# gt1/daccord

Measured on AMD Instinct MI355X. Metric: corrected Mbase/s (whole node), synthetic 20x PacBio piles, higher is better.
Workload: dtype u64+f64; 1 GPU; BASELINE.json configs[1] (10k A-reads x 10 kb x 20x, k=14, one MI355X): synthetic 10000 A-reads x 10000 b x 20x, 15% error (ins 80/del 13.3/sub 6.7), k=14, w=40, a=10, tspace=100; piles_total=10000, piles_rank0=10000, overlaps_rank0=319252, windows_rank0=9969965, trace_blocks_rank0=17906701, corrected_bases_total=90715992

## Files before the change

daccord_amd/csrc/capi.hip:

```cpp
#include <hip/hip_runtime.h>
#include <vector>
#include <string>
#include <cstring>
#include <cstdio>
#include <cstdlib>
#include <new>
#include "../../include/daccord_hip.h"
#include "batch_plan.hpp"
#include "host_tables.hpp"
#include "window_kernels.hpp"
#include "trace_kernel.hpp"
#include "vote_kernel.hpp"
#include "emit_record.hpp"

using namespace dacc;


struct PrepBatch
{
	DevOvl const * ovl; uint64_t novl; uint8_t const * trace; uint32_t trace_bytes;
	uint32_t * blk_ovl; uint32_t * blk_b0;
};

__global__ void k_prep(PrepBatch B)
// ... 323 lines not shown
	std::vector<uint32_t> h_rlen;
	BatchPlan BP;
	DevBuf<DevPile> d_piles; DevBuf<DevOvl> d_ovl; DevBuf<uint32_t> d_ovl_pile; DevBuf<uint8_t> d_trace;
	DevBuf<uint32_t> d_blk_ovl, d_blk_b0, d_wt_b, d_wt_e;
	DevBuf<uint8_t> d_wrec; DevBuf<WindowOut> d_wout; DevBuf<uint8_t> d_arena;
	DevBuf<uint8_t> d_has, d_oc, d_outsym, d_pilebad; DevBuf<uint16_t> d_ld0; DevBuf<uint32_t> d_ocs, d_nfrag, d_err;
	DevBuf<VoteFragment> d_frags; DevBuf<uint64_t> d_fragbase; DevBuf<uint64_t> d_prof;
	DevBuf<uint64_t> d_vst; DevBuf<uint32_t> d_tab32; DevBuf<uint8_t> d_gslab, d_longslab ; DevBuf<uint32_t> d_longhand[2];  DevBuf<uint32_t> d_retry[TIER_NSLOTS], d_work, d_gearly, d_pregen, d_pregen2, d_pregenlist; DevBuf<uint8_t> d_arena2; DevBuf<uint64_t> d_trslab; DevBuf<uint32_t> d_small; DevBuf<uint64_t> d_hand; DevBuf<uint32_t> d_handctr; uint32_t handcap; uint64_t handwant, nruns; bool nohand, oom; bool tier7_adapt_off; int env_t7adapt; int env_trdyn;
	TierSwitches sw; TierPipeline TP;
	struct Stage { bool ran; uint32_t grid; DevBuf<uint32_t> handon; DevBuf<uint8_t> slab; hipEvent_t done; uint32_t const * in;  } st[TIER_NSTAGES];
	uint32_t nlong[2];
	bool longran[2]; hipEvent_t evLong[4];
	uint32_t retry_grid, early_grid; int sched;
	uint32_t tr_grid, tr_lds, tr_words, tr_lanes, trace_bytes, win_grid;
	int env_sched, env_dbgretry;
	std::vector<uint32_t> retry_flags;
	std::vector<dacc_fragment> frags; std::string bases;
	std::vector<int32_t> pile_status; std::vector<std::string> pile_errors; std::string pile_errors_joined;
	std::vector<uint32_t> h_nfrag; std::vector<VoteFragment> h_frags; HostBuf<uint8_t> h_outsym;
	dacc_timing timing;
};

#define HIPCHK(call) do { hipError_t const e_ = (call); if ( e_ != hipSuccess ) { c->err = std::string(#call) + ": " + hipGetErrorString(e_); if ( e_ == hipErrorOutOfMemory ) c->oom = true; return DACC_EHIP; } } while (0)

template<typename T>
static int upload(dacc_ctx * c, DevBuf<T> & b, T const * src, size_t n)
{
	HIPCHK(b.ensure(n ? n : 1));
	if ( n ) HIPCHK(hipMemcpyAsync(b.p,src,n*sizeof(T),hipMemcpyHostToDevice,c->stream));
	return DACC_OK;
// ... 28 lines not shown
	if ( hipGetDeviceCount(&ndev) != hipSuccess || ndev <= 0 || p->device < 0 || p->device >= ndev )
		return DACC_ENODEV;
	if ( hipSetDevice(p->device) != hipSuccess ) return DACC_ENODEV;
	dacc_ctx * c = new (std::nothrow) dacc_ctx;
	if ( !c ) return DACC_ENOMEM;
	c->par = *p; c->device = p->device; c->haveprofile = c->havedb = c->havebatch = false; c->est_cor = 0; c->nlong[0] = c->nlong[1] = 0; c->longran[0] = c->longran[1] = false; c->handcap = 0; c->handwant = 0; c->nruns = 0; c->nohand = false; c->oom = false;
	std::memset(&c->timing,0,sizeof(c->timing));
	c->retry_grid = c->early_grid = c->win_grid = 0; c->tier7_adapt_off = false; c->sched = 0;
	c->tr_grid = c->tr_lds = c->tr_words = c->tr_lanes = c->trace_bytes = 0;
	{
		c->sw = readTierSwitches();
		char const * sc = getenv("DACC_SCHED"); c->env_sched = sc ? atoi(sc) : 1;
		{ char const * td = getenv("DACC_TRACE_DYN"); c->env_trdyn = !(td && td[0] == '0'); }
		char const * ta = getenv("DACC_T7_ADAPT"); c->env_t7adapt = !(ta && ta[0] == '0');
		char const * dr = getenv("DACC_DEBUG_RETRY"); c->env_dbgretry = (dr && dr[0] == '1');
	}
	if ( hipStreamCreate(&c->stream) != hipSuccess ) { delete c; return DACC_EHIP; }
	{ int lo = 0, hi = 0; hipDeviceGetStreamPriorityRange(&lo,&hi); if ( hipStreamCreateWithPriority(&c->stream2,hipStreamNonBlocking,hi) != hipSuccess ) { delete c; return DACC_EHIP; } }
	hipEventCreateWithFlags(&c->evFirstTier,hipEventDisableTiming); hipEventCreateWithFlags(&c->evEarlyGeneric,hipEventDisableTiming); hipEventCreateWithFlags(&c->evPrescan,hipEventDisableTiming);
	for ( int i = 0; i < 6; ++i ) hipEventCreate(&c->ev[i]);
	for ( int i = 0; i < 2; ++i ) hipEventCreate(&c->evEmit[i]);
	for ( int i = 0; i < 4; ++i ) hipEventCreate(&c->evLong[i]);
	for ( int i = 0; i < TIER_NSLOTS; ++i ) hipEventCreate(&c->evslot[i]);
	for ( int i = 0; i < TIER_NSTAGES; ++i ) { hipEventCreate(&c->st[i].done); c->st[i].ran = false; c->st[i].grid = 0; c->st[i].in = 0; }
	*out = c;
	return DACC_OK;
}

void dacc_destroy(dacc_ctx * c)
{
// ... 127 lines not shown
		WB.pregen = 0;
		for ( uint32_t i = 0; i < TIER_NSTAGES; ++i ) c->st[i].ran = false;
		if ( TP.usefast && TP.anytier() )
		{
			HIPCHK(hipMemsetAsync(c->d_pregen.p,0,((BP.nwindows+31)/32+1)*sizeof(uint32_t),s));
			HIPCHK(hipMemsetAsync(c->d_pregen2.p,0,((BP.nwindows+31)/32+1)*sizeof(uint32_t),s));
			HIPCHK(hipMemsetAsync(c->d_pregenlist.p,0,sizeof(uint32_t),s));
			for ( int i = 0; i < TIER_NSLOTS; ++i ) HIPCHK(hipMemsetAsync(c->d_retry[i].p,0,sizeof(uint32_t),s));
			if ( BP.ovl.size() )
			{
				hipLaunchKernelGGL(k_prescan,dim3((BP.ovl.size()+3)/4),dim3(256),0,s,c->d_ovl.p,static_cast<uint64_t>(BP.ovl.size()),c->d_ovl_pile.p,c->d_piles.p,c->d_wt_b.p,c->d_wt_e.p,c->d_pregen.p,c->d_pregen2.p,TP.widetier ? 128u : 64u);
				hipLaunchKernelGGL(k_prescan_lists,dim3(((BP.nwindows+31)/32+255)/256),dim3(256),0,s,c->d_pregen.p,c->d_pregen2.p,static_cast<uint64_t>(BP.nwindows),c->d_pregenlist.p,
					TP.slot1_long ? c->d_retry[0].p : static_cast<uint32_t *>(0),c->d_wout.p);
			}
			HIPCHK(hipEventRecord(c->evPrescan,s));
			FastBatch FL; FL.W = WB; FL.W.arena = c->d_arena2.p; FL.W.prof = 0; FL.W.pregen = 0; FL.F = BP.stageCaps(ID_LONG); FL.dpsq_vst = c->d_vst.p; FL.retry = 0; FL.gearly = 0; FL.gslab = 0; FL.gstride = 0; FL.tab32 = c->d_tab32.p; FL.hand = 0; FL.handctr = 0; FL.handcap = 0; FL.handwords = 0;
#if defined(DACC_LEDGER)
			FL.ledger = 0;
#endif
			bool const long5 = TP.ok[ID_LONG] && TP.tier[ID_LONG] == 5;
			if ( TP.tier[ID_LONG] != 5 ) FL.F = tierCaps(5,c->H.nrows,c->H.nsup);
			if ( !long5 ) FL.F.ldsbytes = 0;
			auto const launchLong = [&](uint32_t const * const lst, uint32_t & nlist, hipEvent_t const filled, uint32_t const which) -> int
			{
				nlist = 0;
				HIPCHK(hipStreamWaitEvent(c->stream2,filled,0));
				HIPCHK(hipMemcpyAsync(&nlist,lst,sizeof(uint32_t),hipMemcpyDeviceToHost,c->stream2));
				HIPCHK(hipStreamSynchronize(c->stream2));
				if ( !nlist ) return DACC_OK;
				uint32_t const * glist = lst;
				if ( TP.ok[ID_LONG] && TP.tier[ID_LONG] != 5 )
// ... 32 lines not shown
			HIPCHK(hipMemsetAsync(c->d_gearly.p,0,sizeof(uint32_t),s));
			HIPCHK(hipMemsetAsync(c->d_handctr.p,0,sizeof(uint32_t),s));
			bool early = false;
			HIPCHK(hipMemsetAsync(c->d_work.p,0,WORK_LONGSTR*sizeof(uint32_t),s));
			auto const work = [&](uint32_t const off) { return (c->sched&1) ? c->d_work.p+off : static_cast<uint32_t *>(0); };
			uint32_t const * list = 0; int lastslot = -1;
			FastBatch FZ;
			for ( uint32_t slot = 0; slot < TIER_NSLOTS; ++slot )
			{
				if ( TP.slotok(slot) )
				{
					int const m = TIER_MAIN[slot];
					FastBatch FB; FB.W = WB; FB.F = BP.stageCaps(m); FB.dpsq_vst = c->d_vst.p; FB.retry = c->d_retry[slot].p;
					if ( (slot > 0 && TP.late_long) || TP.widetier ) FB.W.pregen = c->d_pregen2.p;
					FB.gslab = c->d_gslab.p; FB.gstride = FB.F.gbytes; FB.tab32 = c->d_tab32.p;
					FB.hand = c->handcap ? c->d_hand.p : static_cast<uint64_t *>(0); FB.handctr = c->d_handctr.p; FB.handcap = c->handcap; FB.handwords = TP.handwords;
#if defined(DACC_LEDGER)
					{ char const * lm = getenv("DACC_LEDGER_MASK"); FB.ledger = lm ? static_cast<uint32_t>(strtoul(lm,0,0)) : 0u; }
#endif
					FB.gearly = early ? static_cast<uint32_t *>(0) : c->d_gearly.p;
					int fr[TIER_NSTAGES]; uint32_t nfr = 0;
					for ( int i = 0; i < m; ++i ) if ( TIER_CHAIN[i].slot == slot && TP.ok[i] && !((TIER_CHAIN[i].flags & STAGE_ADAPTIVE) && c->tier7_adapt_off) ) fr[nfr++] = i;
					bool const classed = nfr && (TIER_CHAIN[fr[0]].flags & STAGE_PREPASS);
					if ( classed ) HIPCHK(hipMemsetAsync(c->d_small.p,0,sizeof(uint32_t),s));
					for ( uint32_t k = 0; k < nfr; ++k ) HIPCHK(hipMemsetAsync(c->st[fr[k]].handon.p,0,sizeof(uint32_t),s));
					uint32_t const * in = list;
					if ( classed )
					{
						uint32_t * const mid = c->st[fr[0]].handon.p, * const big = c->st[fr[nfr-1]].handon.p;
						hipLaunchKernelGGL(k_classify,dim3((BP.nwindows+255)/256),dim3(256),0,s,WB,c->d_small.p,mid,big,c->sw.t0inst,nfr > 1 ? c->sw.t7inst : 0u);
						if ( nfr > 1 ) { HIPCHK(hipMemcpyAsync(c->d_work.p+WORK_PRE_MID,mid,sizeof(uint32_t),hipMemcpyDeviceToDevice,s)); HIPCHK(hipMemcpyAsync(c->d_work.p+WORK_PRE_BIG,big,sizeof(uint32_t),hipMemcpyDeviceToDevice,s)); }
// ... 501 lines not shown
```

daccord_amd/csrc/fast_window.hpp:

```cpp
#ifndef DACC_FAST_WINDOW_HPP
#define DACC_FAST_WINDOW_HPP
#include "wave.hpp"
#include "dev_types.hpp"
#include "arena.hpp"
#include "window_main.hpp"
#include "tier_pipeline.hpp"
#include "emit_record.hpp"

namespace dacc {

enum { WS_RETRY = 4 };
enum { FNOPAR = 0xFF };
enum { FSEQCAP = 48 };

struct FSI { uint64_t w; uint16_t left, right, current, path; };
struct FCC { uint64_t w; uint32_t o, l; };

template<int TIER> struct FastTier;
#if !defined(DACC_RCH01)
#define DACC_RCH01 2
#endif
template<> struct FastTier<1> { typedef uint8_t id_t; typedef uint8_t sid_t; enum : uint32_t { smax = 250, gw = 1, wcapg = 1024, rch = DACC_RCH01, fch = 4, fnw = 2, fnc = 40, idmax = 250, rpstcap = 256, lstr = 64, maxs = 32, precap = 1024, ncap = 776, scap = 112, lcap = 960, wcap = 1024, rccap = 144, fcap = 192, siqcap = 56, blcap = 96, seqcap = 32, psiq = 8, consrow = 64, lscrids = 2048, wide = 0, mins = 0, gmem = 0 }; };
template<> struct FastTier<0> { typedef uint8_t id_t; typedef uint8_t sid_t; enum : uint32_t { smax = 250, gw = 1, wcapg = 768, rch = DACC_RCH01, fch = 4, fnw = 2, fnc = 32, idmax = 250, rpstcap = 256, lstr = 64, maxs = 28, precap = 576, ncap = 524, scap = 88, lcap = 640, wcap = 768, rccap = 96, fcap = 128, siqcap = 56, blcap = 96, seqcap = 32, psiq = 8, consrow = 64, lscrids = 2048, wide = 0, mins = 0, gmem = 0 }; };
template<> struct FastTier<7> { typedef uint8_t id_t; typedef uint8_t sid_t; enum : uint32_t { smax = 250, gw = 1, wcapg = 896, rch = DACC_RCH01, fch = 4, fnw = 2, fnc = 32, idmax = 250, rpstcap = 256, lstr = 64, maxs = 28, precap = 704, ncap = 640, scap = 104, lcap = 800, wcap = 896, rccap = 112, fcap = 148, siqcap = 56, blcap = 96, seqcap = 32, psiq = 8, consrow = 64, lscrids = 2048, wide = 0, mins = 0, gmem = 0 }; };
// ... 401 lines not shown
	static_assert(CT::gmem == 0 || CT::gw != 0,"a layout in device memory is the gw layout");
	return C;
}

struct FastBatch
{
	WindowBatch W;
	FastCaps F;
	uint64_t const * dpsq_vst;
	uint32_t * retry;
	uint32_t * gearly;
	uint8_t * gslab;
	uint64_t gstride;
	uint32_t const * tab32;
	uint64_t * hand; uint32_t * handctr; uint32_t handcap, handwords;
#if defined(DACC_LEDGER)
	uint32_t ledger;
#endif
};

template<typename CT>
DEV void fast_load_tables(FastLds<CT> const & L, uint32_t const nrows, uint32_t const nsup, DevTables const & T, uint64_t const * vst)
{
	int const lane = wv_lane();
	for ( uint32_t i = lane; i < nsup; i += WSZ ) { L.suplo8()[i] = T.suplo[i]; L.suphi8()[i] = T.suphi[i]; }
	wv_sync();
}

#if defined(DACC_LEDGER)
#define LEDGER_REP(bit) for ( uint32_t lrep_ = 0, lrn_ = 1u + ((ledger >> (bit)) & 1u); lrep_ < lrn_; ++lrep_ )
// ... 32 lines not shown
	for ( size_t i = 0; i < it.size(); ++i ) tot += it[i];
	for ( size_t i = 0; i < it.size(); i += 64 ) { uint32_t m = 0; for ( size_t q = i; q < it.size() && q < i+64; ++q ) m = std::max(m,it[q]); lock += m; }
	std::vector< std::pair<uint32_t,uint32_t> > P; for ( size_t i = 0; i < it.size(); ++i ) P.push_back(std::make_pair(ln[i],it[i]));
	std::stable_sort(P.begin(),P.end(),[](std::pair<uint32_t,uint32_t> const & a, std::pair<uint32_t,uint32_t> const & b){ return a.first > b.first; });
	for ( size_t i = 0; i < P.size(); i += 64 ) { uint32_t m = 0; for ( size_t q = i; q < P.size() && q < i+64; ++q ) m = std::max(m,P[q].second); locksorted += m; }
	uint64_t lockcls = 0;
	{
		std::vector< std::pair<uint32_t,uint32_t> > Q; for ( size_t i = 0; i < it.size(); ++i ) { uint32_t c = 0; while ( (2u<<c) <= ln[i] ) ++c; Q.push_back(std::make_pair(c,it[i])); }
		std::stable_sort(Q.begin(),Q.end(),[](std::pair<uint32_t,uint32_t> const & a, std::pair<uint32_t,uint32_t> const & b){ return a.first > b.first; });
		for ( size_t i = 0; i < Q.size(); i += 64 ) { uint32_t m = 0; for ( size_t q = i; q < Q.size() && q < i+64; ++q ) m = std::max(m,Q[q].second); lockcls += m; }
	}
	fprintf(f,"%zu %llu %llu %llu %llu\n",it.size(),(unsigned long long)tot,(unsigned long long)lock,(unsigned long long)locksorted,(unsigned long long)lockcls);
	g_feasit.clear();
}
static inline bool feasit_on() { static int on = -1; if ( on < 0 ) on = getenv("DACC_EMUL_FEAS") ? 1 : 0; return on == 1; }
#define FEAS_ITERS(t,len,n) { if ( feasit_on() ) { g_feasit.it.push_back(n); g_feasit.ln.push_back(len); } }
#define FEAS_DUMP() { if ( feasit_on() ) feasit_dump(); }
struct FeasCases
{
	enum { NU = 0, NCU, NTASK, EMPTY_FIRST, EMPTY_MID, EMPTY_LAST, START_AT_ROUND, START_AT_ROUND_END, SPANS_ROUNDS, ROUNDS, LENMASK, MAXLEN, AT_CLAMP, PAST_CLAMP, MULTI, FAIL0, FAIL1, FAILLAST, NODES, N };
	uint64_t v[N];
	void clear() { for ( int i = 0; i < N; ++i ) v[i] = 0; }
	template<typename PT> void units(PT W, uint32_t const nu)
	{
		clear();
		v[NU] = nu;
		uint32_t first = nu, last = 0;
		for ( uint32_t q = 0; q < nu; ++q ) if ( W[q] ) { if ( first == nu ) first = q; last = q; }
		uint64_t t = 0;
		for ( uint32_t q = 0; q < nu; ++q )
		{
			uint32_t const w = W[q];
// ... 12 lines not shown
		if ( j == 0 ) { v[LENMASK] |= 1ull << (len < 63 ? len : 63); if ( len > v[MAXLEN] ) v[MAXLEN] = len; }
		if ( pp+1 == nrows ) ++v[AT_CLAMP];
		if ( pp >= nrows ) ++v[PAST_CLAMP];
		if ( f > 1 ) ++v[MULTI];
	}
	void fail(uint32_t const j, uint32_t const len) { if ( j == 0 ) ++v[FAIL0]; if ( j == 1 ) ++v[FAIL1]; if ( j+1 == len && len > 2 ) ++v[FAILLAST]; }
	void dump(int const tier, uint32_t const nwF, uint32_t const nwR)
	{
		static FILE * f = 0; static bool tried = false;
		if ( !tried ) { tried = true; char const * fn = getenv("DACC_EMUL_FEASCASES"); if ( fn ) f = fopen(fn,"w"); }
		if ( !f ) return;
		fprintf(f,"%d",tier); for ( int i = 0; i < N; ++i ) fprintf(f," %llu",(unsigned long long)v[i]); fprintf(f," %u %u\n",nwF,nwR); fflush(f);
	}
};
static FeasCases g_feascases;
#define FEAS_UNITS(W,nu) { if ( lane == 0 ) g_feascases.units(W,nu); }
#define FEAS_NODE(j,len,pp,nrows,f) g_feascases.node(j,len,pp,nrows,f);
#define FEAS_FAIL(j,len) g_feascases.fail(j,len);
#define FEAS_CASES_DUMP() { if ( lane == 0 ) g_feascases.dump(int(CT::maxs),nwF,nwR); }
#else
#define FEAS_ITERS(t,len,n)
#define FEAS_DUMP()
#define FEAS_UNITS(W,nu)
#define FEAS_NODE(j,len,pp,nrows,f)
#define FEAS_FAIL(j,len)
#define FEAS_CASES_DUMP()
#define FSTAT_MX(i,x)
#define FSTAT_ADD(i,x)
#endif

template<typename CT>
struct FastEngine
{
	typedef typename CT::id_t id_t;
	typedef typename CT::sid_t sid_t;
	enum : uint32_t { SB = 8u*sizeof(sid_t), SMASK = (1u<<SB)-1u, SNONE = SMASK, SMAX = CT::smax };
	FastLds<CT> L; DevTables T; DevParams P;
	uint32_t nrows, nsup;
	uint64_t const * vst;
	enum : bool { GW = (CT::gw != 0) };
	uint8_t * gslab;
	uint32_t const * gtab;
	struct G4 { uint32_t x, y, z, w; };
	int lane; uint32_t flags;
#if defined(DACC_LEDGER)
	uint32_t ledger;
#endif
	uint64_t * prof;
	uint32_t mao, k; uint64_t kmask;
	uint32_t npre, nlast, nn, nmfirst, nmlast;
	uint32_t n0, npool, nlinks, nwF, nwR;
	uint32_t nF, nL;

#if defined(DACC_EMUL)
	DEV void over_(uint32_t b, int line) { flags |= b; static char const * ov = getenv("DACC_EMUL_OVER"); if ( ov ) fprintf(stderr,"[over] tier maxs=%d line %d bits 0x%x nn=%u n0=%u npool=%u nF=%u nL=%u nwF=%u nwR=%u rstop=%u\n",int(CT::maxs)*10000+int(CT::ncap),line,b,nn,n0,npool,nF,nL,nwF,nwR,rstop); }
	#define over(b) over_(b,__LINE__)
#else
	DEV void over(uint32_t b) { flags |= b; }
#endif
#if defined(DACC_PROFILE) && !defined(DACC_EMUL)
	DEV void pcount(int id, uint64_t v) { if ( prof ) atomicAdd(reinterpret_cast<unsigned long long *>(prof+id),static_cast<unsigned long long>(v)); }
	DEV uint64_t pclock() { return clock64(); }
#else
	DEV void pcount(int, uint64_t) {}
	DEV uint64_t pclock() { return 0; }
#endif

#if defined(DACC_PROFILE) && !defined(DACC_EMUL)
// ... 785 lines not shown
			uint32_t const z = L.lnode()[c], par = L.parL()[c];
			if ( z == 0xFFFF ) continue;
			if ( par == SNONE ) ok |= reachN[z];
			else
			{
				ok |= vis[par];
				uint32_t const pl = L.posL()[c];
				for ( uint32_t f = 0; f < nF; ++f ) if ( L.parF()[f] == par && L.posF()[f] < pl ) ok = 1;
			}
		}
		bool const res = wv_any(ok) != 0;
		wv_sync();
		return res;
	}

	DEV void loadTab()
	{
		if constexpr ( GW ) return;
		else {
		uint32_t const stride = nrows+1;
		uint32_t pos = static_cast<uint32_t>(lane) / stride, row = static_cast<uint32_t>(lane) - pos*stride;
		uint32_t const dpos = WSZ / stride, drow = WSZ - dpos*stride;
		for ( uint32_t i = lane; i < stride*(nsup+1); i += WSZ )
		{
			L.tab()[i] = (row < nrows && pos < nsup) ? static_cast<uint32_t>(vst[pos*nrows+row]) : 0u;
			pos += dpos; row += drow; if ( row >= stride ) { row -= stride; ++pos; }
		}
		wv_sync();
		}
	}
	DEV uint32_t tabR(uint32_t const idx) const
	{
		if constexpr ( GW ) return gtab[idx];
		else return L.tab()[idx];
	}
	DEV auto unitRecords() const
	{
		if constexpr ( GW ) return L.urec();
		else { static_assert(2*CT::scap < 512,"unit ids are packed into 9 bits of a 16 bit record"); return reinterpret_cast<LDSQ uint16_t *>(L.ulo()); }
	}
	DEV void computeStretchFeasLanes(uint32_t const sfrom, uint32_t const sto)
	{
		PROFX_T0
		uint32_t const ns = sto-sfrom, nu = 2*ns;
		uint32_t const stride = nrows+1;
		enum { NCHU = (2*CT::scap + WSZ - 1)/WSZ, NCLS = 12 };
		typedef typename FastLds<CT>::toff_t toff_t;
		enum : uint32_t { TOFFMAX = sizeof(toff_t) == 2 ? 0xFFFFu : 0xFFFFFFu };
		static_assert(sizeof(toff_t) == 2 || 2ull*CT::scap*128ull <= TOFFMAX,"task offsets: every (stretch, direction, position) triple can be named");
		auto const urec = unitRecords();
		uint32_t ulo_r[NCHU], uw_r[NCHU], ucls_r[NCHU], upos_r[NCHU];
		#pragma unroll
		for ( uint32_t cc = 0; cc < NCHU; ++cc )
		{
			uint32_t const u = cc*WSZ + lane;
			uint32_t w = 0, lo_ = 0, cls = NCLS;
			if ( u < nu )
			{
				bool const rev = u >= ns; uint32_t const s = sfrom + (rev ? u-ns : u);
				uint32_t const len = L.sslen()[s]; LDSQ uint16_t const * Lk = L.links() + L.slink()[s];
				int32_t lo = 0, hi = static_cast<int32_t>(nrows);
				uint32_t const sh = rev ? 16 : 0;
				for ( uint32_t j = 0; j < len; ++j )
				{
					uint32_t const g = L.nrange()[Lk[rev ? (len-1-j) : j]] >> sh;
					int32_t const jj = static_cast<int32_t>(j);
					int32_t const a = static_cast<int32_t>(g&0xFF)-jj, b = static_cast<int32_t>((g>>8)&0xFF)-jj;
					lo = a > lo ? a : lo; hi = b < hi ? b : hi;
				}
				if ( hi < lo ) hi = lo;
				w = static_cast<uint32_t>(hi-lo); lo_ = static_cast<uint32_t>(lo);
				cls = len >= 49 ? 0u : len >= 33 ? 1u : len >= 25 ? 2u : len >= 17 ? 3u : len >= 13 ? 4u : len >= 9 ? 5u : len >= 7 ? 6u : len >= 5 ? 7u : len == 4 ? 8u : len == 3 ? 9u : len == 2 ? 10u : 11u;
				if ( rev ) { L.maskR()[s] = 0; L.woffR()[s] = 0; } else { L.maskF()[s] = 0; L.woffF()[s] = 0; }
				if constexpr ( CT::wide != 0 ) { if ( rev ) L.maskRh()[s] = 0; else L.maskFh()[s] = 0; }
			}
			ulo_r[cc] = lo_; uw_r[cc] = w; ucls_r[cc] = cls; upos_r[cc] = 0;
		}
		{
			uint32_t run = 0;
			for ( uint32_t k = 0; k < NCLS; ++k )
			{
				#pragma unroll
				for ( uint32_t cc = 0; cc < NCHU; ++cc )
				{
					if ( cc*WSZ >= nu ) break;
					bool const mine = ucls_r[cc] == k;
					uint32_t tot; uint32_t const pre = wv_scan_flag(mine,tot);
					if ( mine ) upos_r[cc] = run + pre;
					run += tot;
				}
			}
		}
		#pragma unroll
		for ( uint32_t cc = 0; cc < NCHU; ++cc )
		{
			uint32_t const u = cc*WSZ + lane;
			if ( u < nu ) { urec[upos_r[cc]] = ulo_r[cc] | (u << 7); L.toff()[upos_r[cc]] = static_cast<toff_t>(uw_r[cc]); }
		}
		wv_sync();
		FEAS_UNITS(L.toff(),nu)
		uint32_t tbase = 0;
		uint32_t ncu = 0;
		for ( uint32_t c = 0; c < nu; c += WSZ )
		{
			uint32_t const q = c + lane;
			uint32_t const w = q < nu ? L.toff()[q] : 0u;
			uint32_t const r = q < nu ? urec[q] : 0u;
			uint32_t tot; uint32_t const pre = wv_scan_excl(w,tot);
			uint32_t ntot; uint32_t const npre = wv_scan_flag(w != 0,ntot);
			if ( w != 0 ) { urec[ncu+npre] = r; L.toff()[ncu+npre] = static_cast<toff_t>(tbase + pre); }
			tbase += tot; ncu += ntot;
		}
		PROFX(18)
		if ( tbase > TOFFMAX ) { over(128); return; }
		if ( lane == 0 ) L.toff()[ncu] = static_cast<toff_t>(tbase);
		wv_sync();
		uint32_t const ntask = tbase;
		uint64_t const ltmask = wv_lanemask_lt();
		uint32_t ubase = 0;
		for ( uint32_t c = 0; c < ntask; c += WSZ )
		{
			uint32_t const t = c + lane;
			bool const act = t < ntask;
			uint32_t u = 0;
			{
				uint32_t const qi = ubase + 1u + static_cast<uint32_t>(lane);
				uint32_t const d = static_cast<uint32_t>(L.toff()[qi < ncu ? qi : ncu]) - c - 1u;
				uint64_t const starts = wv_or64(d < static_cast<uint32_t>(WSZ) ? (1ull << d) : 0ull);
				u = ubase + dacc_popc64(starts & ltmask);
// ... 38 lines not shown
					}
					FEAS_NODE(j,len,pp,nrows,f_a)
					if ( U < FW_THRES_FEAS ) { ok = false; FEAS_ITERS(t,len,j+1) FEAS_FAIL(j,len) break; }
					sum += U;
					if ( j == 0 ) f1 = U;
					fl = U;
					i0_a = i0_b; f_a = f_b; U_a = U_b; i0_b = i0_c; f_b = f_c; ip_b = ip_c; i0_c = i0_d; f_c = f_d; z_d = z_e;
				}
				if ( ok ) { FEAS_ITERS(t,len,len) }
				#undef DACC_LKN
			}
			uint64_t const okb = wv_ballot(ok);
			uint64_t const revb = wv_ballot(act && rev);
			uint64_t const mydir = rev ? revb : ~revb;
			uint32_t const base = rev ? nwR : nwF;
			if ( ok )
			{
				uint32_t const o = base + dacc_popc64(okb & mydir & ltmask);
				if ( o < CT::wcap )
				{
					if ( rev ) putR(o,sum,f1); else putF(o,sum,f1,fl);
				}
			}
			if ( act )
			{
				uint32_t const firstlane = (t0 > c) ? (t0-c) : 0u;
				if ( static_cast<uint32_t>(lane) == firstlane )
				{
					uint32_t const tend = L.toff()[u+1];
					uint32_t const lastlane = (tend-c < WSZ) ? (tend-c) : static_cast<uint32_t>(WSZ);
					uint64_t const span = (lastlane-firstlane >= 64) ? ~0ull : ((1ull << (lastlane-firstlane))-1ull);
					if constexpr ( CT::wide != 0 )
					{
						uint64_t const seg = (okb >> firstlane) & span;
						uint64_t const blo = P < 64u ? (seg << P) : 0ull, bhi = P < 64u ? (P ? (seg >> (64u-P)) : 0ull) : (seg << (P-64u));
						if ( rev ) { L.maskR()[s] |= blo; L.maskRh()[s] |= bhi; } else { L.maskF()[s] |= blo; L.maskFh()[s] |= bhi; }
					}
					else
					{
					uint64_t const bits = ((okb >> firstlane) & span) << P;
					if ( rev ) L.maskR()[s] |= bits; else L.maskF()[s] |= bits;
					}
					if ( t == t0 ) { uint32_t const wo = base + dacc_popc64(okb & mydir & ltmask); if ( rev ) L.woffR()[s] = wo; else L.woffF()[s] = wo; }
				}
			}
			nwF += dacc_popc64(okb & ~revb); nwR += dacc_popc64(okb & revb);
			if ( nwF > CT::wcap || nwR > CT::wcap ) { over(128); FEAS_DUMP() return; }
		}
		FEAS_DUMP()
		wv_sync();
		FEAS_CASES_DUMP()
	}
	enum : uint32_t { FQMAX = FastLds<CT>::fqmax, NWHB = FQMAX <= 255u ? 8u : (FQMAX <= 1023u ? 10u : 12u), NWHMASK = (1u << NWHB) - 1u,
		SWHB = FQMAX <= 1023u ? 16u : 18u, SWHMASK = (1u << SWHB) - 1u };
	static_assert((static_cast<uint64_t>(FQMAX)*0xFFFFFFFFull) >> (32u+NWHB) == 0,"high part of a node weight: fqmax table words");
	static_assert((64ull*static_cast<uint64_t>(FQMAX)*0xFFFFFFFFull) >> (32u+SWHB) == 0,"high part of a stretch weight: 64 nodes");
	static_assert(SWHB + NWHB <= 32u,"reverse record: both high parts in its third word");
	static_assert(SWHB == 16u || FastLds<CT>::wides,"a stretch weight of more than 48 bits needs the 32 byte forward record");
	static_assert(CT::maxs <= 1024 || (FastLds<CT>::fqmax == 4095u && FastLds<CT>::icap == 8u*CT::precap && FastLds<CT>::xwides),"more than 1024 strings: the widths of FastLds<CT>::xwides");
	static_assert(FastLds<CT>::wides || 16u + 2u*NWHB <= 32u,"forward record: three high parts in its fourth word, or the 32 byte record");
	struct G8 { G4 a, b; };
	struct WF { uint64_t w, w1, wl; };
	struct WR { uint64_t w, w1; };
	DEV WF recF(uint32_t const i) const
	{
		WF r;
// ... 71 lines not shown
	{
		if ( p >= nrows ) return 0;
		uint32_t const i0 = L.nps()[z], f = L.nfreq()[z];
		LDSQ uint8_t const * IP = rev ? L.irpos() : L.ipos();
		uint64_t u = 0;
		for ( uint32_t q = 0; q < f; ++q ) u += tabR(static_cast<uint32_t>(IP[i0+q])*(nrows+1) + p);
		return u;
	}
	DEV static bool mask2Test(uint64_t const m0, uint64_t const m1, uint32_t const p) { return p < 64u ? ((m0 >> p) & 1ull) != 0 : ((m1 >> (p-64u)) & 1ull) != 0; }
	DEV static uint32_t mask2Rank(uint64_t const m0, uint64_t const m1, uint32_t const p)
	{
		return p < 64u ? dacc_popc64(m0 & ((1ull<<p)-1ull)) : dacc_popc64(m0) + dacc_popc64(m1 & ((1ull<<(p-64u))-1ull));
	}
	DEV int32_t sfFind(uint32_t const s, uint32_t const p) const
	{
		if constexpr ( CT::wide != 0 )
		{
			if ( p >= 128 ) return -1;
			uint64_t const m0 = L.maskF()[s], m1 = L.maskFh()[s];
			if ( !mask2Test(m0,m1,p) ) return -1;
			return L.woffF()[s] + mask2Rank(m0,m1,p);
		}
		if ( p >= 64 ) return -1;
		uint64_t const m = L.maskF()[s];
		if ( !((m>>p)&1) ) return -1;
		return L.woffF()[s] + dacc_popc64(m & ((1ull<<p)-1));
	}
	DEV int32_t csfFind(uint32_t const s, uint32_t const p) const
	{
		if constexpr ( CT::wide != 0 )
		{
			if ( p >= 128 ) return -1;
			uint64_t const m0 = L.maskR()[s], m1 = L.maskRh()[s];
			if ( !mask2Test(m0,m1,p) ) return -1;
			return L.woffR()[s] + mask2Rank(m0,m1,p);
		}
		if ( p >= 64 ) return -1;
		uint64_t const m = L.maskR()[s];
		if ( !((m>>p)&1) ) return -1;
		return L.woffR()[s] + dacc_popc64(m & ((1ull<<p)-1));
	}
	DEV bool linkOk(uint32_t const i, uint32_t const b) const
	{
		uint32_t const shift = L.sslen()[b]-1;
		if constexpr ( CT::wide != 0 )
		{
			if ( shift >= 128 ) return false;
			uint64_t const a0 = L.maskR()[i], a1 = L.maskRh()[i], b0 = L.maskR()[b], b1 = L.maskRh()[b];
			uint64_t const s0 = shift < 64u ? (b0 << shift) : 0ull;
			uint64_t const s1 = shift < 64u ? ((b1 << shift) | (shift ? (b0 >> (64u-shift)) : 0ull)) : (b0 << (shift-64u));
			uint64_t c0 = a0 & s0, c1 = a1 & s1;
			uint64_t weight = 0;
			while ( c0 | c1 )
			{
				uint32_t pa;
				if ( c0 ) { pa = __builtin_ctzll(c0); c0 &= c0-1; } else { pa = 64u + static_cast<uint32_t>(__builtin_ctzll(c1)); c1 &= c1-1; }
				uint32_t const ia = L.woffR()[i] + mask2Rank(a0,a1,pa);
				uint32_t const pb = pa-shift;
// ... 1407 lines not shown
		LEDGER_REP(6) findCandidatesAndPieces();
		flags = wv_or(flags); if ( flags ) return false;
		nLmagic = nL > 1 ? static_cast<uint32_t>(((1ull<<32) + nL - 1u) / nL) : 0u;
#if !defined(DACC_NO_REACH)
		{
			SITE_T0
			bool reach = false;
			LEDGER_REP(7) reach = pairReachable();
			SITE(23)
			if ( !reach ) { FSTAT_ADD(23,1); PROF(*this,16) return false; }
		}
#endif
		PROF(*this,16)
		loadTab();
		PROF(*this,17)
		LEDGER_REP(8) { nwF = 0; nwR = 0; computeStretchFeasLanes(0,npool); }
		flags = wv_or(flags); if ( flags ) return false;
		{ SITE_T0 bool const sf0_ = sfresh, sd0_ = sdirty; LEDGER_REP(9) { sfresh = sf0_; sdirty = sd0_; spillS(); } SITE(24) }
		PROF(*this,9)

		LEDGER_REP(10)
		{
		if ( lane == 0 ) { L.ctr()[0] = 0; L.ctr()[1] = 0; }
		wv_sync();
		{
			uint32_t sb = 0;
			for ( uint32_t c = 0; c < nL; c += WSZ )
			{
				uint32_t const li = c + lane;
				bool const ract = li < nL;
				REnum R; clInit(R.C,L.rchb() + 8*RNW*lane); R.nrp = 0; R.narp = 0; R.lastk = 0;
				int32_t lastnode = -1;
// ... 269 lines not shown
			{
				uint32_t const e = L.accerr()[c];
				uint32_t rank = 0;
				for ( uint32_t j = 0; j < nc; ++j ) { uint32_t const ej = L.accerr()[j]; rank += (ej < e || (ej == e && j < c)) ? 1u : 0u; }
				ldput(L.ch()+rank,ldget(L.acc()+c));
				serr[rank] = e;
			}
			wv_sync();
			for ( uint32_t c = lane; c < nc; c += WSZ ) { ldput(L.acc()+c,ldget(L.ch()+c)); L.accerr()[c] = serr[c]; }
		}
		wv_sync();
		PROF(*this,13)
		FSTAT_MX(0,mao); FSTAT_MX(1,npre); FSTAT_MX(2,nn); FSTAT_MX(3,n0); FSTAT_MX(4,npool); FSTAT_MX(5,nlinks); FSTAT_MX(6,nwF); FSTAT_MX(7,nwR);
		FSTAT_MX(8,rstop); FSTAT_MX(9,nF); FSTAT_MX(10,nL); FSTAT_ADD(11,1); FSTAT_MX(12,nc); FSTAT_ADD(24,nc ? 0u : 1u);
#if defined(DACC_EMUL)
		if ( lane == 0 ) { FILE * f = ftrav_file(); if ( f ) { uint32_t nlv = 0; for ( uint32_t i = 0; i < nL; ++i ) nlv += L.lnode()[i] != 0xFFFF; fprintf(f,"%d %u %u %u %u %u %u %u %u %u %u %u %u\n",int(CT::maxs),mao,npre,nn,n0,npool,nF,nL,nlv,rstop,nwF,nwR,nc); fflush(f); } }
#endif
		return nc != 0;
	}

	DEV int32_t estimateLength()
	{
		int32_t maxvprodindex = -1;
		uint32_t mn = 0xFFFFFFFFu, mx = 0;
		for ( uint32_t j = lane; j < mao; j += WSZ )
		{
			uint32_t const len = L.slen()[j];
			uint32_t const lastpos = len ? len-1 : 0;
			mn = lastpos < mn ? lastpos : mn; mx = lastpos > mx ? lastpos : mx;
		}
		mn = ~wv_max(~mn); mx = wv_max(mx);
// ... 199 lines not shown
#endif
	if ( B.pregen && ((B.pregen[widx>>5] >> (widx&31)) & 1) ) return FW_DONE;
	E.mao = 0; E.k = 0; E.kmask = 0; E.npre = E.nlast = E.nn = E.nmfirst = E.nmlast = 0; E.n0 = E.npool = E.nlinks = E.nwF = E.nwR = 0; E.nF = E.nL = 0;
	E.nsiq = E.ncdh = E.nacc = 0; E.rstop = 0; E.roundT0 = 0; E.cfree = 0; E.pvpath = E.pvrp = E.pvnf = 0; E.pvcl = 0; E.nmid = 0; E.midbase = 0; E.nLmagic = 0;
	E.T = B.T; E.P = B.P; E.nrows = FB.F.nrows; E.nsup = FB.F.nsup; E.vst = FB.dpsq_vst;
	E.gslab = 0; E.gtab = FB.tab32; E.sfresh = true; E.sdirty = false;
	if ( CT::gw )
	{
#if defined(DACC_EMUL)
		E.gslab = FB.gslab;
#else
		E.gslab = FB.gslab + static_cast<uint64_t>(blockIdx.x)*FB.gstride;
#endif
		if constexpr ( FastOneSlab<CT>::value != 0 ) E.gslab = (uint8_t *)(lds) + FastLds<CT>::g_base;
	}
	E.lane = wv_lane(); E.flags = 0; E.prof = B.prof;
#if defined(DACC_LEDGER)
	E.ledger = FB.ledger;
#endif
#if defined(DACC_PROFILE) && !defined(DACC_EMUL)
	uint64_t * const prof = E.prof;
#endif
#if defined(DACC_EMUL)
	g_fstats.clear();
#endif
	E.L.base = lds;
	FastLds<CT> const & L = E.L;
	int const lane = E.lane;
	PROF_T0
	int32_t curff = B.P.maxff;
	uint32_t hslot = 0;
// ... 245 lines not shown
```

Before: 40.31 Mbase/s.

## Prune stretch feasibility tasks using reachability distances from first/last nodes

Adds a fixed-point pass that computes shortest forward distances from first-window nodes and reverse distances from last-window nodes through the stretch graph. The stretch feasibility task generator then uses these to clamp or drop per-unit position ranges that cannot lie on a path within the length bound, so fewer feasibility tasks are enumerated and stored. It is enabled by default and can be turned off with an environment variable. The cost is an extra iterative wave-synchronous pass per traversal, plus emulator-only auditing code, and the pruning could change results if the distance bounds are wrong.

```diff
diff --git a/daccord_amd/csrc/capi.hip b/daccord_amd/csrc/capi.hip
--- a/daccord_amd/csrc/capi.hip
+++ b/daccord_amd/csrc/capi.hip
@@ -361,6 +361,7 @@
 	uint32_t retry_grid, early_grid; int sched;
 	uint32_t tr_grid, tr_lds, tr_words, tr_lanes, trace_bytes, win_grid;
 	int env_sched, env_dbgretry;
+	uint32_t env_feasneed;
 	std::vector<uint32_t> retry_flags;
 	std::vector<dacc_fragment> frags; std::string bases;
 	std::vector<int32_t> pile_status; std::vector<std::string> pile_errors; std::string pile_errors_joined;
@@ -419,6 +420,7 @@
 		{ char const * td = getenv("DACC_TRACE_DYN"); c->env_trdyn = !(td && td[0] == '0'); }
 		char const * ta = getenv("DACC_T7_ADAPT"); c->env_t7adapt = !(ta && ta[0] == '0');
 		char const * dr = getenv("DACC_DEBUG_RETRY"); c->env_dbgretry = (dr && dr[0] == '1');
+		{ char const * fn = getenv("DACC_FEAS_NEED"); c->env_feasneed = (fn && fn[0] == '0') ? 0u : 1u; }
 	}
 	if ( hipStreamCreate(&c->stream) != hipSuccess ) { delete c; return DACC_EHIP; }
 	{ int lo = 0, hi = 0; hipDeviceGetStreamPriorityRange(&lo,&hi); if ( hipStreamCreateWithPriority(&c->stream2,hipStreamNonBlocking,hi) != hipSuccess ) { delete c; return DACC_EHIP; } }
@@ -576,7 +578,7 @@
 					TP.slot1_long ? c->d_retry[0].p : static_cast<uint32_t *>(0),c->d_wout.p);
 			}
 			HIPCHK(hipEventRecord(c->evPrescan,s));
-			FastBatch FL; FL.W = WB; FL.W.arena = c->d_arena2.p; FL.W.prof = 0; FL.W.pregen = 0; FL.F = BP.stageCaps(ID_LONG); FL.dpsq_vst = c->d_vst.p; FL.retry = 0; FL.gearly = 0; FL.gslab = 0; FL.gstride = 0; FL.tab32 = c->d_tab32.p; FL.hand = 0; FL.handctr = 0; FL.handcap = 0; FL.handwords = 0;
+			FastBatch FL; FL.W = WB; FL.W.arena = c->d_arena2.p; FL.W.prof = 0; FL.W.pregen = 0; FL.F = BP.stageCaps(ID_LONG); FL.dpsq_vst = c->d_vst.p; FL.retry = 0; FL.gearly = 0; FL.gslab = 0; FL.gstride = 0; FL.tab32 = c->d_tab32.p; FL.hand = 0; FL.handctr = 0; FL.handcap = 0; FL.handwords = 0; FL.feasneed = c->env_feasneed;
 #if defined(DACC_LEDGER)
 			FL.ledger = 0;
 #endif
@@ -639,7 +641,7 @@
 					FastBatch FB; FB.W = WB; FB.F = BP.stageCaps(m); FB.dpsq_vst = c->d_vst.p; FB.retry = c->d_retry[slot].p;
 					if ( (slot > 0 && TP.late_long) || TP.widetier ) FB.W.pregen = c->d_pregen2.p;
 					FB.gslab = c->d_gslab.p; FB.gstride = FB.F.gbytes; FB.tab32 = c->d_tab32.p;
-					FB.hand = c->handcap ? c->d_hand.p : static_cast<uint64_t *>(0); FB.handctr = c->d_handctr.p; FB.handcap = c->handcap; FB.handwords = TP.handwords;
+					FB.hand = c->handcap ? c->d_hand.p : static_cast<uint64_t *>(0); FB.handctr = c->d_handctr.p; FB.handcap = c->handcap; FB.handwords = TP.handwords; FB.feasneed = c->env_feasneed;
 #if defined(DACC_LEDGER)
 					{ char const * lm = getenv("DACC_LEDGER_MASK"); FB.ledger = lm ? static_cast<uint32_t>(strtoul(lm,0,0)) : 0u; }
 #endif
diff --git a/daccord_amd/csrc/fast_window.hpp b/daccord_amd/csrc/fast_window.hpp
--- a/daccord_amd/csrc/fast_window.hpp
+++ b/daccord_amd/csrc/fast_window.hpp
@@ -439,6 +439,7 @@
 	uint64_t gstride;
 	uint32_t const * tab32;
 	uint64_t * hand; uint32_t * handctr; uint32_t handcap, handwords;
+	uint32_t feasneed;
 #if defined(DACC_LEDGER)
 	uint32_t ledger;
 #endif
@@ -501,8 +502,8 @@
 	g_feasit.clear();
 }
 static inline bool feasit_on() { static int on = -1; if ( on < 0 ) on = getenv("DACC_EMUL_FEAS") ? 1 : 0; return on == 1; }
-#define FEAS_ITERS(t,len,n) { if ( feasit_on() ) { g_feasit.it.push_back(n); g_feasit.ln.push_back(len); } }
-#define FEAS_DUMP() { if ( feasit_on() ) feasit_dump(); }
+#define FEAS_ITERS(t,len,n) { if ( feasit_on() && !feascount ) { g_feasit.it.push_back(n); g_feasit.ln.push_back(len); } }
+#define FEAS_DUMP() { if ( feasit_on() && !feascount ) feasit_dump(); }
 struct FeasCases
 {
 	enum { NU = 0, NCU, NTASK, EMPTY_FIRST, EMPTY_MID, EMPTY_LAST, START_AT_ROUND, START_AT_ROUND_END, SPANS_ROUNDS, ROUNDS, LENMASK, MAXLEN, AT_CLAMP, PAST_CLAMP, MULTI, FAIL0, FAIL1, FAILLAST, NODES, N };
@@ -545,10 +546,49 @@
 	}
 };
 static FeasCases g_feascases;
-#define FEAS_UNITS(W,nu) { if ( lane == 0 ) g_feascases.units(W,nu); }
-#define FEAS_NODE(j,len,pp,nrows,f) g_feascases.node(j,len,pp,nrows,f);
-#define FEAS_FAIL(j,len) g_feascases.fail(j,len);
-#define FEAS_CASES_DUMP() { if ( lane == 0 ) g_feascases.dump(int(CT::maxs),nwF,nwR); }
+#define FEAS_UNITS(W,nu) { if ( lane == 0 && !feascount ) g_feascases.units(W,nu); }
+#define FEAS_NODE(j,len,pp,nrows,f) { if ( !feascount ) g_feascases.node(j,len,pp,nrows,f); }
+#define FEAS_FAIL(j,len) { if ( !feascount ) g_feascases.fail(j,len); }
+#define FEAS_CASES_DUMP() { if ( lane == 0 && !feascount ) g_feascases.dump(int(CT::maxs),nwF,nwR); }
+struct FeasNeedAudit
+{
+	enum { SCAP = 65536 };
+	uint64_t outF[SCAP][2], outR[SCAP][2];
+	uint64_t ntrav, units0, tasks0, units1, tasks1, recF, recR, probeF, probeR, linkR, insF, insL, mids, hlek, passes;
+	FILE * f; bool tried;
+	bool on() { if ( !tried ) { tried = true; char const * fn = getenv("DACC_EMUL_FEASNEED"); if ( fn ) f = fopen(fn,"w"); } return f != 0; }
+	static void range(uint64_t * m, uint32_t const lo, uint32_t const hi) { for ( uint32_t p = lo; p < hi && p < 128u; ++p ) m[p>>6] |= 1ull << (p&63u); }
+	void unit(uint32_t const s, bool const rev, uint32_t const lo0, uint32_t const hi0, uint32_t const lo1, uint32_t const hi1)
+	{
+		if ( !on() || s >= SCAP ) return;
+		uint64_t * const m = rev ? outR[s] : outF[s];
+		m[0] = m[1] = 0; range(m,lo0,hi0);
+		uint64_t k[2] = {0,0}; range(k,lo1,hi1); m[0] &= ~k[0]; m[1] &= ~k[1];
+		if ( hi0 > lo0 ) { ++units0; tasks0 += hi0-lo0; }
+		if ( hi1 > lo1 ) { ++units1; tasks1 += hi1-lo1; }
+	}
+	static bool out(uint64_t const * m, uint32_t const p) { return p < 128u && ((m[p>>6] >> (p&63u)) & 1ull); }
+	void probe(uint32_t const s, bool const rev, uint32_t const p) { if ( f && s < SCAP && out(rev ? outR[s] : outF[s],p) ) ++(rev ? probeR : probeF); }
+	void link(uint32_t const a, uint32_t const b) { if ( f && a < SCAP && b < SCAP && ((outR[a][0]|outR[a][1]) || (outR[b][0]|outR[b][1])) ) ++linkR; }
+	void dump()
+	{
+		if ( !f ) return;
+		rewind(f);
+		fprintf(f,"%llu %llu %llu %llu %llu %llu %llu %llu %llu %llu %llu %llu %llu %llu %llu\n",(unsigned long long)ntrav,(unsigned long long)units0,(unsigned long long)tasks0,(unsigned long long)units1,(unsigned long long)tasks1,
+			(unsigned long long)recF,(unsigned long long)recR,(unsigned long long)probeF,(unsigned long long)probeR,(unsigned long long)linkR,
+			(unsigned long long)insF,(unsigned long long)insL,(unsigned long long)mids,(unsigned long long)hlek,(unsigned long long)passes);
+		fflush(f);
+	}
+	~FeasNeedAudit() { dump(); }
+};
+static FeasNeedAudit g_feasneed;
+#define FEAS_NEED_UNIT(s,rev,lo0,hi0,lo1,hi1) { if ( !feascount ) g_feasneed.unit(s,rev,lo0,hi0,lo1,hi1); }
+#define FEAS_NEED_PROBE(s,rev,p) g_feasneed.probe(s,rev,p);
+#define FEAS_NEED_LINK(a,b) g_feasneed.link(a,b);
+#define FEAS_OVER() { if ( !feascount ) over(128); }
+#define FEAS_NEED_PASS() { if ( lane == 0 ) ++g_feasneed.passes; }
+#define FEAS_NEED_DUMP() { if ( lane == 0 && !feascount && g_feasneed.on() ) { FeasNeedAudit & A_ = g_feasneed; ++A_.ntrav; A_.recF += nwF; A_.recR += nwR; A_.mids += nmid; A_.hlek += (H <= static_cast<int64_t>(k)); \
+	for ( uint32_t c_ = 0; c_ < nF; ++c_ ) A_.insF += (L.fnode()[c_] != 0xFFFF && L.parF()[c_] != SNONE); for ( uint32_t c_ = 0; c_ < nL; ++c_ ) A_.insL += (L.lnode()[c_] != 0xFFFF && L.parL()[c_] != SNONE); A_.dump(); } }
 #else
 #define FEAS_ITERS(t,len,n)
 #define FEAS_DUMP()
@@ -556,6 +596,12 @@
 #define FEAS_NODE(j,len,pp,nrows,f)
 #define FEAS_FAIL(j,len)
 #define FEAS_CASES_DUMP()
+#define FEAS_NEED_UNIT(s,rev,lo0,hi0,lo1,hi1)
+#define FEAS_NEED_PROBE(s,rev,p)
+#define FEAS_NEED_LINK(a,b)
+#define FEAS_NEED_DUMP()
+#define FEAS_NEED_PASS()
+#define FEAS_OVER() over(128);
 #define FSTAT_MX(i,x)
 #define FSTAT_ADD(i,x)
 #endif
@@ -582,7 +628,15 @@
 	uint32_t npre, nlast, nn, nmfirst, nmlast;
 	uint32_t n0, npool, nlinks, nwF, nwR;
 	uint32_t nF, nL;
-
+	uint32_t feasneed;
+
+#if defined(DACC_EMUL)
+	bool feascount, feasapplied; uint32_t nwFall, nwRall;
+	DEV bool feasNeedOn() const { char const * e = getenv("DACC_FEAS_NEED"); return !(e && e[0] == '0'); }
+#else
+	static constexpr bool feascount = false;
+	DEV bool feasNeedOn() const { return feasneed != 0; }
+#endif
 #if defined(DACC_EMUL)
 	DEV void over_(uint32_t b, int line) { flags |= b; static char const * ov = getenv("DACC_EMUL_OVER"); if ( ov ) fprintf(stderr,"[over] tier maxs=%d line %d bits 0x%x nn=%u n0=%u npool=%u nF=%u nL=%u nwF=%u nwR=%u rstop=%u\n",int(CT::maxs)*10000+int(CT::ncap),line,b,nn,n0,npool,nF,nL,nwF,nwR,rstop); }
 	#define over(b) over_(b,__LINE__)
@@ -1398,6 +1452,46 @@
 		return res;
 	}
 
+	enum : uint32_t { FEASINF = 255u };
+	DEV void feasDistances()
+	{
+		LDSQ uint8_t * const dF = L.xreach();
+		LDSQ uint8_t * const dR = dF + CT::ncap;
+		for ( uint32_t z = lane; z < nn; z += WSZ ) { dF[z] = FEASINF; dR[z] = FEASINF; }
+		wv_sync();
+		for ( uint32_t c = lane; c < nF; c += WSZ ) { uint32_t const z = L.fnode()[c]; if ( z != 0xFFFF ) dF[z] = 0; }
+		for ( uint32_t c = lane; c < nL; c += WSZ ) { uint32_t const z = L.lnode()[c]; if ( z != 0xFFFF ) dR[z] = 0; }
+		wv_sync();
+		while ( true )
+		{
+			uint32_t changed = 0;
+			for ( uint32_t c = lane; c < nF; c += WSZ )
+			{
+				uint32_t const par = L.parF()[c];
+				if ( L.fnode()[c] == 0xFFFF || par == SNONE ) continue;
+				uint32_t const l = L.slast()[par], d = L.sslen()[par]-1u-L.posF()[c];
+				if ( d < dF[l] ) { dF[l] = d; changed = 1; }
+			}
+			for ( uint32_t c = lane; c < nL; c += WSZ )
+			{
+				uint32_t const par = L.parL()[c];
+				if ( L.lnode()[c] == 0xFFFF || par == SNONE ) continue;
+				uint32_t const f = L.sfirst()[par], d = L.posL()[c];
+				if ( d < dR[f] ) { dR[f] = d; changed = 1; }
+			}
+			for ( uint32_t s = lane; s < n0; s += WSZ )
+			{
+				uint32_t const f = L.sfirst()[s], l = L.slast()[s], step = L.sslen()[s]-1u;
+				uint32_t const a = dF[f] + step, b = dR[l] + step;
+				if ( a < dF[l] ) { dF[l] = a; changed = 1; }
+				if ( b < dR[f] ) { dR[f] = b; changed = 1; }
+			}
+			wv_sync();
+			FEAS_NEED_PASS()
+			if ( !wv_any(changed) ) break;
+		}
+	}
+
 	DEV void loadTab()
 	{
 		if constexpr ( GW ) return;
@@ -1423,17 +1517,22 @@
 		if constexpr ( GW ) return L.urec();
 		else { static_assert(2*CT::scap < 512,"unit ids are packed into 9 bits of a 16 bit record"); return reinterpret_cast<LDSQ uint16_t *>(L.ulo()); }
 	}
-	DEV void computeStretchFeasLanes(uint32_t const sfrom, uint32_t const sto)
+	DEV void computeStretchFeasLanes(uint32_t const sfrom, uint32_t const sto, int64_t const lmax, bool const need)
 	{
 		PROFX_T0
 		uint32_t const ns = sto-sfrom, nu = 2*ns;
 		uint32_t const stride = nrows+1;
+		int64_t const H = (lmax+1)/2;
+		int32_t const hcap = H < 1 ? 1 : (H < static_cast<int64_t>(nrows) ? static_cast<int32_t>(H) : static_cast<int32_t>(nrows));
+		LDSQ uint8_t const * const dF = L.xreach();
+		LDSQ uint8_t const * const dR = dF + CT::ncap;
 		enum { NCHU = (2*CT::scap + WSZ - 1)/WSZ, NCLS = 12 };
 		typedef typename FastLds<CT>::toff_t toff_t;
 		enum : uint32_t { TOFFMAX = sizeof(toff_t) == 2 ? 0xFFFFu : 0xFFFFFFu };
 		static_assert(sizeof(toff_t) == 2 || 2ull*CT::scap*128ull <= TOFFMAX,"task offsets: every (stretch, direction, position) triple can be named");
 		auto const urec = unitRecords();
 		uint32_t ulo_r[NCHU], uw_r[NCHU], ucls_r[NCHU], upos_r[NCHU];
+		uint32_t allF = 0, allR = 0;
 		#pragma unroll
 		for ( uint32_t cc = 0; cc < NCHU; ++cc )
 		{
@@ -1453,10 +1552,27 @@
 					lo = a > lo ? a : lo; hi = b < hi ? b : hi;
 				}
 				if ( hi < lo ) hi = lo;
-				w = static_cast<uint32_t>(hi-lo); lo_ = static_cast<uint32_t>(lo);
+				if ( need )
+				{
+					w = static_cast<uint32_t>(hi-lo) << 8; lo_ = static_cast<uint32_t>(lo) << 8;
+					if ( rev ) allR += static_cast<uint32_t>(hi-lo); else allF += static_cast<uint32_t>(hi-lo);
+					if ( !rev ) hi = hi < hcap ? hi : hcap;
+					if ( s < n0 )
+					{
+						int32_t const d = rev ? dR[L.slast()[s]] : dF[L.sfirst()[s]];
+						bool const wanted = rev ? (d == 0 || static_cast<int64_t>(d) + static_cast<int64_t>(k) < H) : true;
+						if ( !rev ) lo = d > lo ? d : lo;
+						if ( d == static_cast<int32_t>(FEASINF) || !wanted ) hi = 0;
+					}
+					if ( hi <= lo ) { lo = 0; hi = 0; }
+				}
+				w |= static_cast<uint32_t>(hi-lo); lo_ |= static_cast<uint32_t>(lo);
 				cls = len >= 49 ? 0u : len >= 33 ? 1u : len >= 25 ? 2u : len >= 17 ? 3u : len >= 13 ? 4u : len >= 9 ? 5u : len >= 7 ? 6u : len >= 5 ? 7u : len == 4 ? 8u : len == 3 ? 9u : len == 2 ? 10u : 11u;
+				if ( !feascount )
+				{
 				if ( rev ) { L.maskR()[s] = 0; L.woffR()[s] = 0; } else { L.maskF()[s] = 0; L.woffF()[s] = 0; }
 				if constexpr ( CT::wide != 0 ) { if ( rev ) L.maskRh()[s] = 0; else L.maskFh()[s] = 0; }
+				}
 			}
 			ulo_r[cc] = lo_; uw_r[cc] = w; ucls_r[cc] = cls; upos_r[cc] = 0;
 		}
@@ -1475,11 +1591,22 @@
 				}
 			}
 		}
+		bool filt = false;
+		if ( need ) { uint32_t const tF = wv_sum(allF), tR = wv_sum(allR); filt = tF <= CT::wcap && tR <= CT::wcap && static_cast<uint64_t>(tF) + tR <= TOFFMAX; }
+	#if defined(DACC_EMUL)
+		if ( !feascount ) feasapplied = filt;
+	#endif
 		#pragma unroll
 		for ( uint32_t cc = 0; cc < NCHU; ++cc )
 		{
 			uint32_t const u = cc*WSZ + lane;
-			if ( u < nu ) { urec[upos_r[cc]] = ulo_r[cc] | (u << 7); L.toff()[upos_r[cc]] = static_cast<toff_t>(uw_r[cc]); }
+			if ( u < nu )
+			{
+				uint32_t const usel = (need && !filt) ? 8u : 0u, umask = need ? 0xFFu : ~0u;
+				uint32_t const wsel = (uw_r[cc] >> usel) & umask, lsel = (ulo_r[cc] >> usel) & umask;
+				FEAS_NEED_UNIT(sfrom + (u >= ns ? u-ns : u),u >= ns,need ? (ulo_r[cc] >> 8) : lsel,need ? (ulo_r[cc] >> 8) + (uw_r[cc] >> 8) : lsel+wsel,lsel,lsel+wsel)
+				urec[upos_r[cc]] = lsel | (u << 7); L.toff()[upos_r[cc]] = static_cast<toff_t>(wsel);
+			}
 		}
 		wv_sync();
 		FEAS_UNITS(L.toff(),nu)
@@ -1496,7 +1623,7 @@
 			tbase += tot; ncu += ntot;
 		}
 		PROFX(18)
-		if ( tbase > TOFFMAX ) { over(128); return; }
+		if ( tbase > TOFFMAX ) { FEAS_OVER() return; }
 		if ( lane == 0 ) L.toff()[ncu] = static_cast<toff_t>(tbase);
 		wv_sync();
 		uint32_t const ntask = tbase;
@@ -1565,7 +1692,7 @@
 			uint64_t const revb = wv_ballot(act && rev);
 			uint64_t const mydir = rev ? revb : ~revb;
 			uint32_t const base = rev ? nwR : nwF;
-			if ( ok )
+			if ( ok && !feascount )
 			{
 				uint32_t const o = base + dacc_popc64(okb & mydir & ltmask);
 				if ( o < CT::wcap )
@@ -1573,7 +1700,7 @@
 					if ( rev ) putR(o,sum,f1); else putF(o,sum,f1,fl);
 				}
 			}
-			if ( act )
+			if ( act && !feascount )
 			{
 				uint32_t const firstlane = (t0 > c) ? (t0-c) : 0u;
 				if ( static_cast<uint32_t>(lane) == firstlane )
@@ -1596,11 +1723,12 @@
 				}
 			}
 			nwF += dacc_popc64(okb & ~revb); nwR += dacc_popc64(okb & revb);
-			if ( nwF > CT::wcap || nwR > CT::wcap ) { over(128); FEAS_DUMP() return; }
+			if ( nwF > CT::wcap || nwR > CT::wcap ) { FEAS_OVER() FEAS_DUMP() return; }
 		}
 		FEAS_DUMP()
 		wv_sync();
 		FEAS_CASES_DUMP()
+		FEAS_NEED_DUMP()
 	}
 	enum : uint32_t { FQMAX = FastLds<CT>::fqmax, NWHB = FQMAX <= 255u ? 8u : (FQMAX <= 1023u ? 10u : 12u), NWHMASK = (1u << NWHB) - 1u,
 		SWHB = FQMAX <= 1023u ? 16u : 18u, SWHMASK = (1u << SWHB) - 1u };
@@ -1702,6 +1830,7 @@
 	}
 	DEV int32_t sfFind(uint32_t const s, uint32_t const p) const
 	{
+		FEAS_NEED_PROBE(s,false,p)
 		if constexpr ( CT::wide != 0 )
 		{
 			if ( p >= 128 ) return -1;
@@ -1716,6 +1845,7 @@
 	}
 	DEV int32_t csfFind(uint32_t const s, uint32_t const p) const
 	{
+		FEAS_NEED_PROBE(s,true,p)
 		if constexpr ( CT::wide != 0 )
 		{
 			if ( p >= 128 ) return -1;
@@ -1730,6 +1860,7 @@
 	}
 	DEV bool linkOk(uint32_t const i, uint32_t const b) const
 	{
+		FEAS_NEED_LINK(i,b)
 		uint32_t const shift = L.sslen()[b]-1;
 		if constexpr ( CT::wide != 0 )
 		{
@@ -3167,8 +3298,17 @@
 		PROF(*this,16)
 		loadTab();
 		PROF(*this,17)
-		LEDGER_REP(8) { nwF = 0; nwR = 0; computeStretchFeasLanes(0,npool); }
+		LEDGER_REP(8) { nwF = 0; nwR = 0; bool const need = feasNeedOn(); if ( need ) feasDistances(); computeStretchFeasLanes(0,npool,lmax,need); }
 		flags = wv_or(flags); if ( flags ) return false;
+#if defined(DACC_EMUL)
+		nwFall = nwF; nwRall = nwR;
+		if ( ftrav_file() && feasapplied )
+		{
+			uint32_t const kF = nwF, kR = nwR;
+			feascount = true; nwF = 0; nwR = 0; computeStretchFeasLanes(0,npool,lmax,false); feascount = false;
+			nwFall = nwF; nwRall = nwR; nwF = kF; nwR = kR;
+		}
+#endif
 		{ SITE_T0 bool const sf0_ = sfresh, sd0_ = sdirty; LEDGER_REP(9) { sfresh = sf0_; sdirty = sd0_; spillS(); } SITE(24) }
 		PROF(*this,9)
 
@@ -3468,7 +3608,7 @@
 		FSTAT_MX(0,mao); FSTAT_MX(1,npre); FSTAT_MX(2,nn); FSTAT_MX(3,n0); FSTAT_MX(4,npool); FSTAT_MX(5,nlinks); FSTAT_MX(6,nwF); FSTAT_MX(7,nwR);
 		FSTAT_MX(8,rstop); FSTAT_MX(9,nF); FSTAT_MX(10,nL); FSTAT_ADD(11,1); FSTAT_MX(12,nc); FSTAT_ADD(24,nc ? 0u : 1u);
 #if defined(DACC_EMUL)
-		if ( lane == 0 ) { FILE * f = ftrav_file(); if ( f ) { uint32_t nlv = 0; for ( uint32_t i = 0; i < nL; ++i ) nlv += L.lnode()[i] != 0xFFFF; fprintf(f,"%d %u %u %u %u %u %u %u %u %u %u %u %u\n",int(CT::maxs),mao,npre,nn,n0,npool,nF,nL,nlv,rstop,nwF,nwR,nc); fflush(f); } }
+		if ( lane == 0 ) { FILE * f = ftrav_file(); if ( f ) { uint32_t nlv = 0; for ( uint32_t i = 0; i < nL; ++i ) nlv += L.lnode()[i] != 0xFFFF; fprintf(f,"%d %u %u %u %u %u %u %u %u %u %u %u %u\n",int(CT::maxs),mao,npre,nn,n0,npool,nF,nL,nlv,rstop,nwFall,nwRall,nc); fflush(f); } }
 #endif
 		return nc != 0;
 	}
@@ -3698,7 +3838,10 @@
 #endif
 		if constexpr ( FastOneSlab<CT>::value != 0 ) E.gslab = (uint8_t *)(lds) + FastLds<CT>::g_base;
 	}
-	E.lane = wv_lane(); E.flags = 0; E.prof = B.prof;
+	E.lane = wv_lane(); E.flags = 0; E.prof = B.prof; E.feasneed = FB.feasneed;
+#if defined(DACC_EMUL)
+	E.feascount = false; E.feasapplied = false; E.nwFall = E.nwRall = 0;
+#endif
 #if defined(DACC_LEDGER)
 	E.ledger = FB.ledger;
 #endif
```

Result: faster. 41.82 Mbase/s (median of 6 runs) (+3.7%).
